# Luh1124/face-vae

Hardware: AMD Instinct MI355X
Metric: training images/sec (256x256 face-VAE step) (higher is better)
Workload: dtype bf16; 1 GPU; FaceVAE step 256x256 (AFE trunk + reparam + Generator trunk, MSE+KL, Adam); global_batch=32, per_gpu_batch=32, resolution=256, parallelism=dp1

## Files before the change

face-vae_amd/csrc/conv.hip:

```cpp
#include "conv_plan.h"

namespace {

#ifdef FV_DIAG
constexpr int DIAG_SLOTS = 8;
__device__ unsigned long long g_diag[4096 * 8 * DIAG_SLOTS];
#define FV_DIAG_T(var) const unsigned long long var = __builtin_amdgcn_s_memtime()
#define FV_DIAG_PUT(slot, val)                                                                     \
  do {                                                                                             \
    const unsigned long long v_ = (val);                                                           \
    if ((threadIdx.x & 63) == 0 && blockIdx.x < 4096)                                              \
      g_diag[((size_t)blockIdx.x * (blockDim.x >> 6) + (threadIdx.x >> 6)) * DIAG_SLOTS + (slot)] = v_; \
  } while (0)
#define FV_DIAG_BEGIN()                                                \
  FV_DIAG_T(d_t0);                                                     \
  const unsigned long long d_r0 = __builtin_amdgcn_s_memrealtime();    \
  unsigned long long d_tw = 0, d_ti = 0, d_wb = 0
#define FV_DIAG_PROLOGUE() FV_DIAG_T(d_t1)
#define FV_DIAG_WAIT_BEGIN() FV_DIAG_T(d_wa)
#define FV_DIAG_WAIT_END()                   \
  do {                                       \
    d_wb = __builtin_amdgcn_s_memtime();     \
    d_tw += d_wb - d_wa;                     \
  } while (0)
// ... 142 lines not shown
  auto bcnt = [&](int j) { return j < nsteps ? (2 * j + 1 < ntap ? 2 : 1) * JB : 0; };
  issue_b(0, 0);
  issue_halo(0);
  if (nch > 1) issue_halo(1);
  for (int i = 1; i < NSB - 1; ++i)
    if (i < nsteps) issue_b(i, i);
  wait_vm<0>();
  __syncthreads();
  FV_DIAG_PROLOGUE();
  int pend = 0;
  if (NSB - 1 < nsteps) {
    issue_b(NSB - 1, NSB - 1);
    pend = bcnt(NSB - 1);
  }
  load_frags(fa0, fb0, 0, 0);
  int hn = 2, hstep = (9 * 2 - 10) / 2;
  int bj = 0;
  for (int j = 0; j + 1 < nsteps; ++j) {
    load_frags(fa1, fb1, 2 * j + 1, bj);
    mfma_all(fa0, fb0);
    const int bn1 = bj + 1 == NSB ? 0 : bj + 1;
    FV_DIAG_WAIT_BEGIN();
    if constexpr (NSB == 2) wait_vm<0>();
    else if (pend == 2 * JB) wait_vm<2 * JB>();
    else wait_vm_dyn(pend);
    wait_lgkm0();
    __builtin_amdgcn_s_barrier();
    asm volatile("" ::: "memory");
    FV_DIAG_WAIT_END();
    if (hn < nch && j == hstep) {
      issue_halo(hn);
      ++hn;
      hstep = (9 * hn - 10) / 2;
    }
    pend = 0;
    if (j + NSB < nsteps) {
      issue_b(j + NSB, bj);
      pend = bcnt(j + NSB);
    }
    load_frags(fa0, fb0, 2 * j + 2, bn1);
    FV_DIAG_ISSUE_END();
    mfma_all(fa1, fb1);
    bj = bn1;
  }
  {
    const int j = nsteps - 1;
    const bool two = 2 * j + 1 < ntap;
    load_frags(fa1, fb1, two ? 2 * j + 1 : 2 * j, bj);
    mfma_all(fa0, fb0);
    if (two) mfma_all(fa1, fb1);
  }
  FV_DIAG_LOOP_END();
  __syncthreads();
  conv_epilogue<bf16, WN, WM, RN, RM, true>(a, acc, smem, co0, p0, tm, wn, wm, lane, tid);
  FV_DIAG_END();
}

template <int WM, int RM, typename Mid = NoMid>
__device__ __forceinline__ void subpix_epilogue(const ConvArgs& a, f32x4 (&acc)[4][RM], char* smem, int tn, int n,
                                                int h0, int w0, int tm, int wn, int wm, int lane, int tid,
                                                Mid mid = Mid{}) {
  constexpr bool kMid = !std::is_same<Mid, NoMid>::value;
  constexpr int RN = 4, NT = 64 * 4 * WM, BN = 256, BM = WM * RM * 16, CPR = BN / 8;
  const int lr = lane & 15, lh = lane >> 4;
  const int cb0 = tn * 64;
#pragma unroll
  for (int nn = 0; nn < RN; ++nn)
#pragma unroll
    for (int i = 0; i < 4; ++i) {
      const int co = cb0 + nn * 16 + lh * 4 + i;
      const float bv = a.bias ? a.bias[co] : 0.f;
#pragma unroll
      for (int m = 0; m < RM; ++m) acc[nn][m][i] += bv;
    }
  if (a.stats) {
    const int rec = (tm * WM + wm) * 4 + wn;
#pragma unroll
    for (int nn = 0; nn < RN; ++nn) {
      float sv[4], qv[4];
#pragma unroll
      for (int i = 0; i < 4; ++i) {
        float t = 0.f, q = 0.f;
#pragma unroll
        for (int m = 0; m < RM; ++m) {
          t += acc[nn][m][i];
          q += acc[nn][m][i] * acc[nn][m][i];
        }
        sv[i] = row16_sum(t);
        qv[i] = row16_sum(q);
      }
      const int cb = cb0 + nn * 16 + lh * 4;
      const int ii = lr & 3;
      const float s01 = ii & 1 ? sv[1] : sv[0], s23 = ii & 1 ? sv[3] : sv[2];
      const float q01 = ii & 1 ? qv[1] : qv[0], q23 = ii & 1 ? qv[3] : qv[2];
      const float val = lr < 4 ? (ii & 2 ? s23 : s01) : (ii & 2 ? q23 : q01);
      if (lr < 8 && rec < a.nrec) a.stats[(long)(rec * 2 + (lr >> 2)) * a.Cout + cb + ii] = val;
    }
  }
  __syncthreads();
#pragma unroll
  for (int nn = 0; nn < RN; ++nn) {
    const int cl = wn * 64 + nn * 16 + lh * 4;
#pragma unroll
    for (int m = 0; m < RM; ++m) {
      const int pl = wm * RM * 16 + m * 16 + lr;
      bf16 t4[4] = {(bf16)acc[nn][m][0], (bf16)acc[nn][m][1], (bf16)acc[nn][m][2], (bf16)acc[nn][m][3]};
      char* dst = smem + pl * BN * 2 + (((cl >> 3) ^ (pl & (CPR - 1))) << 4) + ((cl & 4) << 1);
// ... 205 lines not shown
    auto step_barrier = [&]() {
      FV_DIAG_WAIT_BEGIN();
      if constexpr (NSB == 2) wait_vm<0>();
      else if (pend == 2 * JB) wait_vm<2 * JB>();
      else wait_vm_dyn(pend);
      wait_lgkm0();
      __builtin_amdgcn_s_barrier();
      asm volatile("" ::: "memory");
      FV_DIAG_WAIT_END();
    };
    for (int j = 0; j + 1 < nsteps; ++j) {
      load_frags(fa1, fb1, 2 * j + 1, bj);
      if constexpr ((SCH & 2) != 0) {
        if (stag) step_barrier();
      }
      mfma_all(fa0, fb0);
      const int bn1 = bj + 1 == NSB ? 0 : bj + 1;
      if (!stag) step_barrier();
      if (hn < nch && j == hstep) {
        issue_halo(hn);
        ++hn;
        hstep = halo_step(hn);
      }
      pend = 0;
      if (j + NSB < nsteps) {
        issue_b(t.wbase, j + NSB, bj);
        pend = bcnt(j + NSB);
      }
      load_frags(fa0, fb0, 2 * j + 2, bn1);
      FV_DIAG_ISSUE_END();
      mfma_all(fa1, fb1);
      bj = bn1;
    }
    load_frags(fa1, fb1, 2 * nsteps - 1, bj);
    mfma_all(fa0, fb0);
    mfma_all(fa1, fb1);
    if constexpr (SCH & 1) __builtin_amdgcn_s_setprio(0);
    FV_DIAG_LOOP_END();
    __syncthreads();
    const int vn = v + (int)gridDim.x;
    const bool nxt = PERS && vn < ntl;
    const Tile cur = t;
    if constexpr (PERS) {
      auto mid = [&]() {
        if (nxt) {
          t = tile_of(vn);
          mk_hoff(t);
          issue_prologue(t);
        }
      };
      if constexpr (MODE == 1)
        subpix_epilogue<WM, RM>(a, acc, smem, cur.tn, cur.n, cur.th * TR, cur.tw * 64, cur.tm, wn, wm, lane, tid, mid);
      else
        conv_epilogue<bf16, WN, WM, RN, RM, true>(a, acc, smem, cur.co0, cur.p0, cur.tm, wn, wm, lane, tid, mid);
    } else {
      if constexpr (MODE == 1)
        subpix_epilogue<WM, RM>(a, acc, smem, cur.tn, cur.n, cur.th * TR, cur.tw * 64, cur.tm, wn, wm, lane, tid);
      else
        conv_epilogue<bf16, WN, WM, RN, RM, true>(a, acc, smem, cur.co0, cur.p0, cur.tm, wn, wm, lane, tid);
    }
    FV_DIAG_END();
    if (!nxt) break;
    v = vn;
    first = false;
  }
}

template <int KS, int CIN, int RN, int TR, bool WLDS, bool KSPLIT>
__global__ void __launch_bounds__(512, 4)
conv_halo_fwd(ConvArgs a, unsigned x_bytes) {
  constexpr int PAD = KS / 2, TW = 64;
  constexpr int MT = TR * 4;
  constexpr int RM = KSPLIT ? MT : MT / 8;
  constexpr int HR = TR + KS - 1, HW = TW + KS - 1;
  constexpr int CPP = CIN / 8;
  constexpr int HCH = HR * HW * CPP;
  constexpr int HQ = (HCH + 63) / 64;
  constexpr int KPAD = ((KS * KS * CIN + 31) / 32) * 32;
  constexpr int NKS = KPAD / 32;
  constexpr int KPW = (NKS + 7) / 8;
  constexpr int WROW = KPAD / 8 + 1;
  constexpr int WCH = RN * 16 * WROW;
  constexpr int WQ = WLDS ? (WCH + 63) / 64 : 0;
  constexpr int HB = HQ * 1024, WB = WQ * 1024;
  constexpr int SCR = 4096;
  static_assert(!KSPLIT || (RN == 1 && !WLDS && 8 * MT * 1024 <= HB), "k-split layout");
  __shared__ __attribute__((aligned(1024))) char smem[HB + WB + SCR];
  char* halo = smem;
  char* wlds = smem + HB;

  const int tid = threadIdx.x, lane = tid & 63;
  const int wave = __builtin_amdgcn_readfirstlane(tid >> 6);
  const int tiles_w = a.W / TW, tiles_h = a.H / TR;
  const int tile = blockIdx.x;
  const int n = tile / (tiles_h * tiles_w);
  const int rem = tile - n * tiles_h * tiles_w;
  const int h0 = (rem / tiles_w) * TR, w0 = (rem % tiles_w) * TW;
  const int li = lane & 15, g = lane >> 4;
  const bf16* __restrict__ wk = reinterpret_cast<const bf16*>(a.w);

  const __amdgpu_buffer_rsrc_t xr = __builtin_amdgcn_make_buffer_rsrc(const_cast<void*>(a.x), 0, (int)x_bytes, 0x00020000);
  for (int q = wave; q < HQ; q += 8) {
    const int L = q * 64 + lane;
    const int hp = L / CPP, ch = L - (L / CPP) * CPP;
    const int hr = hp / HW, hc = hp - (hp / HW) * HW;
    const int hh = h0 + hr - PAD, ww = w0 + hc - PAD;
    const int sc = ch ^ (hp & (CPP - 1));
    const bool ok = L < HCH && hh >= 0 && hh < a.H && ww >= 0 && ww < a.W;
    const unsigned off = ok ? (unsigned)((((n * a.H + hh) * a.W + ww) * CIN + sc * 8) * 2) : 0x80000000u;
    dma16(xr, halo + q * 1024, off);
  }
  if constexpr (WLDS) {
// ... 1511 lines not shown
  for (int i = 0; i < n; ++i) {
    const fv_conv_desc* d = &descs[i];
    int st = check_desc(d);
    if (st) return st;
    FV_REQUIRE(d->dtype == dtype, "weight_prep_multi: one dtype per call");
    FV_REQUIRE(fv_conv_weight_prep_batchable(d), "weight_prep_multi: conv %d needs a special layout", i);
    FV_REQUIRE(w_params[i] && wks[i], "weight_prep_multi: null pointer (conv %d)", i);
    const int ks = d->ksize;
    WPrepMJob j0{w_params[i], sigmas[i], wks[i], wrows(d->cout), kpad_lay(smaj_wk(d), kpad_of(ks, d->cin)),
                 fv_ilog2(d->cin),
                 ks * ks * d->cin, 0, 0, d->cout, d->cin_valid, ks, 0, smaj_wk(d)};
    j0.nb = (int)std::min<long>(fv_cdiv((long)j0.rows * j0.Kpad, 256), 256);
    nb_total = std::max(nb_total, j0.nb);
    m.j[m.n++] = j0;
    if (wts[i]) {
      const int cin_t = pad_pow2_8(d->cout);
      WPrepMJob j1{w_params[i], sigmas[i], wts[i], wrows(d->cin), kpad_lay(smaj_wt(d), kpad_of(ks, cin_t)),
                   fv_ilog2(cin_t),
                   ks * ks * cin_t, 1, 0, d->cout, d->cin_valid, ks, 0, smaj_wt(d)};
      j1.nb = (int)std::min<long>(fv_cdiv((long)j1.rows * j1.Kpad, 256), 256);
      nb_total = std::max(nb_total, j1.nb);
      m.j[m.n++] = j1;
    }
  }
  hipStream_t s = (hipStream_t)stream;
  if (dtype == FV_BF16)
    hipLaunchKernelGGL(weight_prep_multi_kernel<bf16>, dim3(nb_total, m.n), dim3(256), 0, s, m);
  else
    hipLaunchKernelGGL(weight_prep_multi_kernel<float>, dim3(nb_total, m.n), dim3(256), 0, s, m);
  return fv_check_launch("weight_prep_multi");
}

static int sr_geometry(const fv_conv_desc* d, int* bp) {
  if (d->dtype != FV_BF16 || use_c7n(d) || halo_tr(d) || use_subpix(d) || use_c64(d)) return 0;
  const int bn = halo3_bn(d);
  const long P = (long)d->n * d->h * d->w;
  if (!bn || d->cout % bn || P % 256) return 0;
  const int nw = bn == 64 ? 4 : 8;
  if (bp) *bp = 256 / nw;
  return (int)(P / 256 * nw);
}

extern "C++" {
static int cu_count() {
  static int n = 0;
  if (!n) {
    int dev = 0;
    if (hipGetDevice(&dev) != hipSuccess || hipDeviceGetAttribute(&n, hipDeviceAttributeMultiprocessorCount, dev) != hipSuccess ||
        n <= 0)
      n = 256;
  }
  return n;
}
template <int WN, int WM, int RN, int RM, int NSB, int MODE>
static void launch_h3(int ntiles, hipStream_t s, const ConvArgs& a, unsigned xb) {
  const int sch = res_sched(2) >= 2 ? 2 : 0;
  const char* e = getenv("FV_PERS_GRID");
  const int cap = (e && atoi(e) > 0) ? atoi(e) : cu_count();
  const bool pers = WN * RN * 16 < 256 && ntiles > cap;
  const dim3 g(pers ? cap : ntiles), b(64 * WN * WM);
  if constexpr (WN * RN * 16 < 256) {
    if (pers) {
      if (sch == 2) hipLaunchKernelGGL((conv3_halo_fwd3<WN, WM, RN, RM, NSB, 2, MODE, true>), g, b, 0, s, a, xb, ntiles);
      else hipLaunchKernelGGL((conv3_halo_fwd3<WN, WM, RN, RM, NSB, 0, MODE, true>), g, b, 0, s, a, xb, ntiles);
      return;
    }
  }
  {
    if (sch == 2) hipLaunchKernelGGL((conv3_halo_fwd3<WN, WM, RN, RM, NSB, 2, MODE, false>), g, b, 0, s, a, xb, ntiles);
    else hipLaunchKernelGGL((conv3_halo_fwd3<WN, WM, RN, RM, NSB, 0, MODE, false>), g, b, 0, s, a, xb, ntiles);
  }
}
}

static bool use_c1s(const fv_conv_desc* d) {
  const char* e = getenv("FV_C1S");
  if (e && e[0] == '0') return false;
  if (!use_v2(d) || d->ksize != 1 || d->upsample || d->pro_act) return false;
  if ((d->cin != 256 && d->cin != 512) || d->cout % 256 || d->ldy != d->cout) return false;
  const long P = (long)d->n * d->h * d->w;
  return P % (32768 / d->cin) == 0 && P * d->cout * 2 < (1L << 31);
}

static int conv_run(const fv_conv_desc* d, const void* x, const void* wk, const float* bias,
                    const float* psc, const float* psh, const void* res, void* y, float* stats,
                    hipStream_t s, const fv_store_reduce* sr = nullptr) {
  ConvArgs a{};
  if (sr && sr->mode) {
    FV_REQUIRE(sr_geometry(d, nullptr) > 0, "store-pass records not available for this conv (query fv_conv2d_sr_records)");
    FV_REQUIRE(sr->records, "store-pass records: null buffer");
    FV_REQUIRE(sr->mode == 1 || (sr->mode == 2 && sr->bn_input && sr->mean && sr->invstd && sr->gamma && sr->beta && !res),
               "store-pass records: bad mode / BN arguments");
    FV_REQUIRE(!stats, "store-pass records and accumulator statistics in one call are not supported");
    a.spm = sr->mode;
    a.sprec = sr->records;
    a.bnm = sr->mean; a.bni = sr->invstd; a.bng = sr->gamma; a.bnb = sr->beta; a.bns = sr->slope;
    if (sr->mode == 2) res = sr->bn_input;
  }
  const FwdTile t = fwd_tile(d->cout);
  a.x = x; a.w = wk; a.bias = bias; a.psc = psc; a.psh = psh; a.slope = d->pro_slope;
  a.res = res; a.y = y; a.stats = stats;
  a.nrec = stats ? fv_conv2d_stats_blocks(d) : 0;
  a.N = d->n; a.H = d->h; a.W = d->w;
  a.Hin = d->upsample ? d->h / 2 : d->h;
  a.Win = d->upsample ? d->w / 2 : d->w;
  a.P = d->n * d->h * d->w;
// ... 56 lines not shown
    const int hl = d->h / 2, wl = d->w / 2;
    const long base = (long)d->n * (wl / 32) * (d->cout / 64);
    int nb = 1;
    while (base * nb < 256 && hl % (nb * 16) == 0) nb *= 2;
    const int nblk = (int)(base * nb);
    const unsigned xb = (unsigned)((long)d->n * hl * wl * 128 * 2);
    hipLaunchKernelGGL(conv3up_band_fwd, dim3(nblk), dim3(512), 0, s, a, xb, nb);
    return fv_check_launch("conv2d_fwd_upband");
  }
  if (use_subpix_halo(d)) {
    FV_REQUIRE(!res && !a.spm, "sub-pixel conv: no residual / store-pass records");
    a.H = a.Hin; a.W = a.Win;
    a.Ho = d->h; a.Wo = d->w;
    a.P = d->n * a.H * a.W;
    a.lgtw = 6;
    a.wus = 4 * d->cout * 64;
    a.ntn = d->cout / 64;
    const int nblk = a.ntn * d->n * (a.H / 4) * (a.W / 64);
    const unsigned xb = (unsigned)((long)d->n * a.H * a.W * d->cin * 2);
    FV_REQUIRE((long)4 * (d->cin / 32) * a.wus / 2 <= phase_wk_elems(d), "sub-pixel halo conv: weight image");
    launch_h3<4, 2, 4, 8, 2, 1>(nblk, s, a, xb);
    return fv_check_launch("conv2d_fwd_subpix_halo");
  }
  if (use_subpix(d)) {
    FV_REQUIRE(!res, "sub-pixel conv: no residual");
    const FwdTile t2 = fwd_tile_v2(d->cout);
    a.H = a.Hin; a.W = a.Win;
    a.Ho = d->h; a.Wo = d->w;
    a.P = d->n * a.H * a.W;
    a.lgw = fv_ilog2(a.W); a.lghw = fv_ilog2(a.H * a.W);
    a.Kpad = kpad_of(2, d->cin);
    a.nks = a.Kpad / BK2;
    a.ntn = fv_cdiv(d->cout, t2.bn);
    a.wphase = wrows(d->cout) * a.Kpad;
    if ((st = wext(4L * a.ntn * t2.bn, a.Kpad, "subpix"))) return st;
    const int nblk2 = 4 * a.ntn * (a.P / t2.bm);
    const long xb = (long)d->n * a.Hin * a.Win * d->cin * 2;
    st = launch_v2(a, 2, t2, 2, nblk2, (unsigned)xb, s);
    if (st) {
      fv_set_error("sub-pixel conv variant unsupported (cout=%d)", d->cout);
      return st;
    }
    return fv_check_launch("conv2d_fwd_subpix");
  }
  if (const int bn = c64 ? 0 : halo3_bn(d)) {
    FV_REQUIRE(!(res && stats), "conv v2: residual and BN statistics in one call are not supported");
    a.lgtw = 6;
    a.wus = wk_rows(d) * 64;
    a.ntn = d->cout / bn;
    if ((st = wext(a.ntn * bn, 9L * d->cin, "halo3")) || (st = wext(wk_rows(d), 9L * d->cin, "halo3 units")))
      return st;
    const int nblk = a.ntn * d->n * (d->h / 4) * (d->w / 64);
    const unsigned xb = (unsigned)((long)d->n * d->h * d->w * d->cin * 2);
    if (bn >= 128 && a.Cin % 64 == 0) {
      if (bn == 256) launch_h3<4, 2, 4, 8, 2, 0>(nblk, s, a, xb);
      else launch_h3<2, 4, 4, 4, 3, 0>(nblk, s, a, xb);
    } else if (bn == 256) {
      hipLaunchKernelGGL((conv3_halo_fwd2<4, 2, 4, 8, 2>), dim3(nblk), dim3(512), 0, s, a, xb);
    } else if (bn == 128) {
      hipLaunchKernelGGL((conv3_halo_fwd2<2, 4, 4, 4, 3>), dim3(nblk), dim3(512), 0, s, a, xb);
    } else if (d->h % 8 == 0 && a.Cin % 64 == 0) {
      const int nblk8 = a.ntn * d->n * (d->h / 8) * (d->w / 64);
      launch_h3<1, 8, 4, 4, 2, 0>(nblk8, s, a, xb);
    } else {
      hipLaunchKernelGGL((conv3_halo_fwd2<1, 4, 4, 4, 3>), dim3(nblk), dim3(256), 0, s, a, xb);
    }
    return fv_check_launch("conv2d_fwd_halo3");
  }
  if (use_c1s(d) && !res && !stats && !a.spm) {
    if ((st = wext(d->cout, a.Kpad, "c1s"))) return st;
    FV_REQUIRE(a.Kpad == d->cin, "1x1 stream conv: K %d != Kpad %d", d->cin, a.Kpad);
    const int ncg = d->cout / 256;
    const int grid = std::max(8 * ncg, cu_count() / (8 * ncg) * (8 * ncg));
    const unsigned xb = (unsigned)((long)a.P * d->cin * 2);
    const char* e = getenv("FV_C1S_BP");
    const bool big = e && atoi(e) == 128;
    if (d->cin == 256) {
      if (big) hipLaunchKernelGGL((conv1x1_stream<256, 128>), dim3(grid), dim3(512), 0, s, a, xb);
      else hipLaunchKernelGGL((conv1x1_stream<256, 64>), dim3(grid), dim3(512), 0, s, a, xb);
    } else {
      if (big) hipLaunchKernelGGL((conv1x1_stream<512, 64>), dim3(grid), dim3(512), 0, s, a, xb);
      else hipLaunchKernelGGL((conv1x1_stream<512, 32>), dim3(grid), dim3(512), 0, s, a, xb);
    }
    return fv_check_launch("conv2d_fwd_c1s");
  }
  if (use_v2(d)) {
    FV_REQUIRE(!(res && stats), "conv v2: residual and BN statistics in one call are not supported");
    const FwdTile t2 = fwd_tile_v2(d->cout);
    a.ntn = fv_cdiv(d->cout, t2.bn);
    a.nks = a.Kpad / BK2;
    if ((st = wext((long)a.ntn * t2.bn, a.Kpad, "v2"))) return st;
    const int nblk2 = a.ntn * fv_cdiv(a.P, t2.bm);
    const long xb = (long)d->n * a.Hin * a.Win * d->cin * 2;
    st = launch_v2(a, d->ksize, t2, d->upsample, nblk2, (unsigned)xb, s);
    if (st) {
      fv_set_error("conv v2 variant unsupported (k=%d ups=%d)", d->ksize, d->upsample);
      return st;
    }
    return fv_check_launch("conv2d_fwd_v2");
  }
  const int nblk = a.ntn * fv_cdiv(a.P, t.bm);
  if ((st = wext((long)a.ntn * t.bn, a.Kpad, "v1"))) return st;
  st = d->dtype == FV_BF16 ? launch_fwd<bf16>(a, d->ksize, t, d->pro_act, d->upsample, nblk, s)
                           : launch_fwd<float>(a, d->ksize, t, d->pro_act, d->upsample, nblk, s);
  if (st) {
    fv_set_error("conv variant unsupported (k=%d pro=%d ups=%d)", d->ksize, d->pro_act, d->upsample);
// ... 42 lines not shown
}

int fv_conv2d_sr_records(const fv_conv_desc* d, int dgrad, int* record_pixels) {
  if (check_desc(d) != FV_OK) return 0;
  if (dgrad) {
    if (d->upsample) return 0;
    const fv_conv_desc t = dgrad_desc(d);
    return sr_geometry(&t, record_pixels);
  }
  return sr_geometry(d, record_pixels);
}

int fv_conv2d_fwd_sr(const fv_conv_desc* d, const void* x, const void* wk, const float* bias, const void* res, void* y,
                     const fv_store_reduce* sr, void* stream) {
  int st = check_desc(d);
  if (st) return st;
  FV_REQUIRE(x && wk && y && sr && sr->mode == 1, "fwd_sr: null pointer or mode != 1");
  FV_REQUIRE(!d->pro_act && !d->out_nchw_f32 && d->ldy == d->cout, "fwd_sr: plain NHWC output only");
  return conv_run(d, x, wk, bias, nullptr, nullptr, res, y, nullptr, (hipStream_t)stream, sr);
}

int fv_conv2d_bwd_data_sr(const fv_conv_desc* d, const void* dy, int ldy_dy, const void* wt, void* dx,
                          const fv_store_reduce* sr, void* stream) {
  int st = check_desc(d);
  if (st) return st;
  FV_REQUIRE(dy && wt && dx && sr && sr->mode == 2 && !d->upsample, "bwd_data_sr: bad argument");
  const fv_conv_desc t = dgrad_desc(d);
  FV_REQUIRE(ldy_dy == t.cin, "bwd_data: dy channel stride must be %d (got %d)", t.cin, ldy_dy);
  return conv_run(&t, dy, wt, nullptr, nullptr, nullptr, nullptr, dx, nullptr, (hipStream_t)stream, sr);
}

int fv_conv2d_bwd_data(const fv_conv_desc* d, const void* dy, int ldy_dy, const void* wt, void* dx,
                       void* stream) {
  int st = check_desc(d);
  if (st) return st;
  const fv_conv_desc t = dgrad_desc(d);
  FV_REQUIRE(ldy_dy == t.cin, "bwd_data: dy channel stride must be %d (got %d)", t.cin, ldy_dy);
  if (const int bn = dgrad_halo_bn(d)) {
    FV_REQUIRE(dy && wt && dx, "null pointer");
    ConvArgs a{};
    a.x = dy; a.w = wt; a.y = dx;
    a.N = d->n; a.H = d->h / 2; a.W = d->w / 2; a.Hin = d->h; a.Win = d->w;
    a.Ho = a.H; a.Wo = a.W;
    a.P = d->n * a.H * a.W;
    a.Cin = 4 * d->cout;
    a.K = d->cout;
    a.Cout = d->cin; a.ldy = d->cin;
    a.lgtw = 6;
    a.wus = d->cin * 64;
    a.ntn = d->cin / bn;
    const int nblk = a.ntn * d->n * (a.H / 4) * (a.W / 64);
    const unsigned xb = (unsigned)((long)d->n * d->h * d->w * d->cout * 2);
    FV_REQUIRE((long)(a.Cin / 32) * 4 * a.wus / 2 <= phase_wt_elems(d), "low-res halo dgrad: weight image");
    if (bn == 256) launch_h3<4, 2, 4, 8, 2, 2>(nblk, (hipStream_t)stream, a, xb);
    else launch_h3<2, 4, 4, 4, 3, 2>(nblk, (hipStream_t)stream, a, xb);
    return fv_check_launch("conv2d_bwd_data_lowres_halo");
  }
  if (use_dgrad_lowres(d)) {
    FV_REQUIRE(dy && wt && dx, "null pointer");
    ConvArgs a{};
    const FwdTile t2 = fwd_tile_v2(d->cin);
    a.x = dy; a.w = wt; a.y = dx;
    a.N = d->n; a.H = d->h / 2; a.W = d->w / 2; a.Hin = d->h; a.Win = d->w;
    a.Ho = a.H; a.Wo = a.W;
    a.P = d->n * a.H * a.W;
    a.Cin = t.cin; a.lgCin = fv_ilog2(t.cin);
    a.Cout = d->cin; a.ldy = d->cin;
    a.Kpad = 16 * t.cin; a.K = a.Kpad; a.nks = a.Kpad / BK2;
    a.ntn = fv_cdiv(d->cin, t2.bn);
    const int nblk = a.ntn * fv_cdiv(a.P, t2.bm);
    const long xb = (long)d->n * d->h * d->w * t.cin * 2;
    const int st = launch_v2(a, 4, t2, 3, nblk, (unsigned)xb, (hipStream_t)stream);
    if (st) {
      fv_set_error("low-res dgrad variant unsupported (cin=%d)", d->cin);
      return st;
    }
    return fv_check_launch("conv2d_bwd_data_lowres");
  }
  return conv_run(&t, dy, wt, nullptr, nullptr, nullptr, nullptr, dx, nullptr, (hipStream_t)stream);
}

int fv_conv2d_wgrad_nsplit(const fv_conv_desc* d) {
  if (check_desc(d) != FV_OK) return 0;
  return plan_wgrad(d).nsplit;
}

size_t fv_conv2d_wgrad_slab_elems(const fv_conv_desc* d) {
  if (check_desc(d) != FV_OK) return 0;
  const WgPlan p = plan_wgrad(d);
  return (size_t)(p.sub ? 4 : 1) * p.nsplit * p.CW * p.KW;
}

size_t fv_conv2d_wgrad_bias_slab_elems(const fv_conv_desc* d) {
  if (check_desc(d) != FV_OK) return 0;
  const WgPlan p = plan_wgrad(d);
  return (size_t)(p.sub ? 4 : 1) * p.nsplit * p.CW;
}

int fv_conv2d_bwd_weight(const fv_conv_desc* d, const void* x, const float* pro_scale,
                         const float* pro_shift, const void* dy, int ldy_dy, float* slab,
                         float* bias_slab, void* stream) {
  int st = check_desc(d);
  if (st) return st;
  FV_REQUIRE(x && dy && slab, "null pointer");
  FV_REQUIRE(ldy_dy % 8 == 0 && ldy_dy >= d->cout, "wgrad: dy channel stride must be a multiple of 8 >= cout");
  FV_REQUIRE(!d->pro_act || (pro_scale && pro_shift), "prologue needs scale/shift");
// ... 1384 lines not shown
```

face-vae_amd/csrc/conv_common.h:

```cpp
#pragma once
#include <stdlib.h>

#include <algorithm>
#include <type_traits>

#include "common.h"

#pragma GCC visibility push(hidden)

struct ConvArgs {
  const void* x;
  const void* w;
  const float* bias;
  const float* psc;
  const float* psh;
  float slope;
  const void* res;
  void* y;
  float* stats;
  int N, H, W, Hin, Win, P;
  int lgCin, Cin;
  int Cout, ldy;
  int K, Kpad, nks;
  int sigmoid, nchw;
// ... 49 lines not shown
}

template <typename T>
__device__ __forceinline__ void load4(const T* p, float* f);
template <>
__device__ __forceinline__ void load4<float>(const float* p, float* f) {
  float4 v = *reinterpret_cast<const float4*>(p);
  f[0] = v.x; f[1] = v.y; f[2] = v.z; f[3] = v.w;
}
template <>
__device__ __forceinline__ void load4<bf16>(const bf16* p, float* f) {
  uint2 v = *reinterpret_cast<const uint2*>(p);
  f[0] = __uint_as_float(v.x << 16); f[1] = __uint_as_float(v.x & 0xffff0000u);
  f[2] = __uint_as_float(v.y << 16); f[3] = __uint_as_float(v.y & 0xffff0000u);
}
template <typename T>
__device__ __forceinline__ void store4(T* p, const float* f);
template <>
__device__ __forceinline__ void store4<float>(float* p, const float* f) {
  *reinterpret_cast<float4*>(p) = make_float4(f[0], f[1], f[2], f[3]);
}
template <>
__device__ __forceinline__ void store4<bf16>(bf16* p, const float* f) {
  bf16 t[4] = {(bf16)f[0], (bf16)f[1], (bf16)f[2], (bf16)f[3]};
  *reinterpret_cast<uint2*>(p) = *reinterpret_cast<const uint2*>(t);
}

template <typename T>
struct Frag;
template <>
struct Frag<bf16> {
  bf16x8 v;
  __device__ __forceinline__ void lds(const char* p) { v = *reinterpret_cast<const bf16x8*>(p); }
};
template <>
struct Frag<float> {
  float v[8];
  __device__ __forceinline__ void lds(const char* p) {
    float4 a = reinterpret_cast<const float4*>(p)[0];
    float4 b = reinterpret_cast<const float4*>(p)[1];
    v[0] = a.x; v[1] = a.y; v[2] = a.z; v[3] = a.w;
    v[4] = b.x; v[5] = b.y; v[6] = b.z; v[7] = b.w;
  }
};
__device__ __forceinline__ f32x4 mma(const Frag<bf16>& a, const Frag<bf16>& b, f32x4 c) {
  return __builtin_amdgcn_mfma_f32_16x16x32_bf16(a.v, b.v, c, 0, 0, 0);
}
__device__ __forceinline__ f32x4 mma(const Frag<float>& a, const Frag<float>& b, f32x4 c) {
#pragma unroll
  for (int j = 0; j < 8; ++j) c = __builtin_amdgcn_mfma_f32_16x16x4f32(a.v[j], b.v[j], c, 0, 0, 0);
  return c;
}

struct NoMid {
  __device__ void operator()() const {}
};
template <typename T, int WN, int WM, int RN, int RM, bool STAGED = false, typename Mid = NoMid, bool GSUB = false>
__device__ __forceinline__ void conv_epilogue(const ConvArgs& a, f32x4 (&acc)[RN][RM], char* smem, int co0, int p0,
                                              int tm, int wn, int wm, int lane, int tid, Mid mid = Mid{}) {
  constexpr bool kMid = !std::is_same<Mid, NoMid>::value;
  constexpr int NT = 64 * WN * WM;
  constexpr int BN = WN * RN * 16;
  constexpr int BM = WM * RM * 16;
  const int HW = a.H * a.W;
  const int lr = lane & 15, lh = lane >> 4;
  constexpr int SCPR = BN / 8, NRES = STAGED ? (BM * SCPR + NT - 1) / NT : 1;
  uint4 rpre[NRES];
  auto load_res = [&]() {
    if (a.res) {
#pragma unroll
      for (int it = 0; it < NRES; ++it) {
        const int idx = tid + it * NT;
        const int pl = idx / SCPR, ch = idx - (idx / SCPR) * SCPR;
        const int tp = a.lgtw ? p0 + (pl >> a.lgtw) * a.W + (pl & ((1 << a.lgtw) - 1)) : p0 + pl;
        const int co = co0 + ch * 8;
        rpre[it] = make_uint4(0, 0, 0, 0);
        if (idx < BM * SCPR && tp < a.P && co < a.Cout)
          rpre[it] = *reinterpret_cast<const uint4*>(reinterpret_cast<const bf16*>(a.res) +
                                                      (long)out_pix<GSUB>(a, tp) * a.ldy + co);
      }
    }
  };
  if constexpr (STAGED && !kMid) load_res();
  float bv[RN][4];
#pragma unroll
  for (int n = 0; n < RN; ++n)
#pragma unroll
    for (int i = 0; i < 4; ++i) {
      const int co = co0 + wn * RN * 16 + n * 16 + lh * 4 + i;
      bv[n][i] = (a.bias && co < a.Cout) ? a.bias[co] : 0.f;
    }
  bool pv[RM];
  int pix_of[RM];
#pragma unroll
  for (int m = 0; m < RM; ++m) {
    const int loc = wm * RM * 16 + m * 16 + lr;
    const int tp = a.lgtw ? p0 + (loc >> a.lgtw) * a.W + (loc & ((1 << a.lgtw) - 1)) : p0 + loc;
    pv[m] = tp < a.P;
    pix_of[m] = out_pix<GSUB>(a, tp);
  }
#pragma unroll
  for (int n = 0; n < RN; ++n) {
    const int cb = co0 + wn * RN * 16 + n * 16 + lh * 4;
#pragma unroll
    for (int m = 0; m < RM; ++m) {
#pragma unroll
      for (int i = 0; i < 4; ++i) acc[n][m][i] += bv[n][i];
      if (!STAGED && a.res && pv[m]) {
        const T* rp = reinterpret_cast<const T*>(a.res) + (long)pix_of[m] * a.ldy + cb;
        if (cb + 3 < a.Cout) {
          float f[4];
          load4<T>(rp, f);
#pragma unroll
          for (int i = 0; i < 4; ++i) acc[n][m][i] += f[i];
        } else {
#pragma unroll
          for (int i = 0; i < 4; ++i)
            if (cb + i < a.Cout) acc[n][m][i] += Elt<T>::to_f(rp[i]);
        }
      }
    }
  }

  const long pout = a.Ho ? (long)a.N * a.Ho * a.Wo : (long)a.P;
  if (a.stats && (long)(tm * WM + wm) < (pout + RM * 16 - 1) / (RM * 16) && tm * WM + wm < a.nrec) {
    const int rec = tm * WM + wm;
#pragma unroll
    for (int n = 0; n < RN; ++n) {
      float sv[4], qv[4];
#pragma unroll
      for (int i = 0; i < 4; ++i) {
        float t = 0.f, q = 0.f;
#pragma unroll
        for (int m = 0; m < RM; ++m) {
          const float v = pv[m] ? acc[n][m][i] : 0.f;
          t += v;
          q += v * v;
        }
        sv[i] = row16_sum(t);
        qv[i] = row16_sum(q);
      }
      const int cb = co0 + wn * RN * 16 + n * 16 + lh * 4;
      const int ii = lr & 3;
      const float s01 = ii & 1 ? sv[1] : sv[0], s23 = ii & 1 ? sv[3] : sv[2];
      const float q01 = ii & 1 ? qv[1] : qv[0], q23 = ii & 1 ? qv[3] : qv[2];
      const float val = lr < 4 ? (ii & 2 ? s23 : s01) : (ii & 2 ? q23 : q01);
      if (lr < 8 && cb + ii < a.Cout) a.stats[(long)(rec * 2 + (lr >> 2)) * a.Cout + cb + ii] = val;
    }
  }

  if constexpr (STAGED) {
    static_assert(sizeof(T) == 2, "staged epilogue is bf16 NHWC");
    constexpr int CPR = BN / 8;
    __syncthreads();
#pragma unroll
    for (int n = 0; n < RN; ++n) {
      const int cl = wn * RN * 16 + n * 16 + lh * 4;
#pragma unroll
      for (int m = 0; m < RM; ++m) {
        const int pl = wm * RM * 16 + m * 16 + lr;
        bf16 t4[4] = {(bf16)acc[n][m][0], (bf16)acc[n][m][1], (bf16)acc[n][m][2], (bf16)acc[n][m][3]};
        char* dst = smem + pl * BN * 2 + (((cl >> 3) ^ (pl & (CPR - 1))) << 4) + ((cl & 4) << 1);
        *reinterpret_cast<uint2*>(dst) = *reinterpret_cast<const uint2*>(t4);
      }
    }
    __syncthreads();
    uint4 vv[kMid ? NRES : 1];
    if constexpr (kMid) {
#pragma unroll
      for (int it = 0; it < NRES; ++it) {
        const int idx = tid + it * NT;
        const int pl = idx / CPR, ch = idx - (idx / CPR) * CPR;
        if (idx < BM * CPR) vv[it] = *reinterpret_cast<const uint4*>(smem + pl * BN * 2 + ((ch ^ (pl & (CPR - 1))) << 4));
      }
      __syncthreads();
      load_res();
      mid();
    }
    auto chunk = [&](int it, int pl, int ch) -> uint4 {
      if constexpr (kMid) return vv[it];
      else return *reinterpret_cast<const uint4*>(smem + pl * BN * 2 + ((ch ^ (pl & (CPR - 1))) << 4));
    };
    if (!a.spm) {
#pragma unroll
      for (int it = 0; it < NRES; ++it) {
        const int idx = tid + it * NT;
        if (idx >= BM * CPR) break;
        const int pl = idx / CPR, ch = idx - (idx / CPR) * CPR;
        const int tp = a.lgtw ? p0 + (pl >> a.lgtw) * a.W + (pl & ((1 << a.lgtw) - 1)) : p0 + pl;
        const int co = co0 + ch * 8;
        if (tp >= a.P || co >= a.Cout) continue;
        const int pix = out_pix<GSUB>(a, tp);
        Chunk8<bf16> v;
        v.raw = chunk(it, pl, ch);
        T* yp = reinterpret_cast<T*>(a.y) + (long)pix * a.ldy + co;
        if (a.res) {
          Chunk8<bf16> r;
          r.raw = rpre[it];
          float f[8];
#pragma unroll
          for (int j = 0; j < 8; ++j) f[j] = v.get(j) + r.get(j);
          v.set8(f);
        }
        v.store(reinterpret_cast<bf16*>(yp));
      }
      return;
    }
    const int sch = tid % CPR;
    float sacc[8], qacc[8], bm_[8], bi_[8], bg_[8], bb_[8];
#pragma unroll
    for (int j = 0; j < 8; ++j) sacc[j] = qacc[j] = 0.f;
    if (a.spm == 2) {
      const int c = co0 + sch * 8;
#pragma unroll
      for (int j = 0; j < 8; ++j) {
        const bool ok = c + j < a.Cout;
        bm_[j] = ok ? a.bnm[c + j] : 0.f;
        bi_[j] = ok ? a.bni[c + j] : 0.f;
        bg_[j] = ok ? a.bng[c + j] : 0.f;
        bb_[j] = ok ? a.bnb[c + j] : 0.f;
      }
    }
#pragma unroll
    for (int it = 0; it < NRES; ++it) {
      const int idx = tid + it * NT;
      if (idx >= BM * CPR) break;
      const int pl = idx / CPR, ch = idx - (idx / CPR) * CPR;
      const int tp = a.lgtw ? p0 + (pl >> a.lgtw) * a.W + (pl & ((1 << a.lgtw) - 1)) : p0 + pl;
      const int co = co0 + ch * 8;
      if (tp >= a.P || co >= a.Cout) continue;
      const int pix = out_pix<GSUB>(a, tp);
      Chunk8<bf16> v;
      v.raw = chunk(it, pl, ch);
      T* yp = reinterpret_cast<T*>(a.y) + (long)pix * a.ldy + co;
      Chunk8<bf16> r;
// ... 143 lines not shown
```

Baseline: 2667 images/s.

## Specialize halo conv epilogue with precomputed addresses and fused store-pass BN statistics

Adds a HALO template path to the staged conv epilogue for whole-tile halo 3x3 convolutions. It precomputes per-thread global and LDS addresses, drops bounds checks, fetches bias once per lane and broadcasts it with ds_bpermute, and folds residual add, BN-backward reductions and per-channel stats into a single store pass using packed float2 math. The goal is less integer address arithmetic and fewer branches in the epilogue. Host-side requirements now reject shapes that are not whole tiles, which could turn previously supported shapes into errors.

Measured after the change: 2715 images/s (median of 6 runs). 1.02x the previous value.

```diff
diff --git a/face-vae_amd/csrc/conv.hip b/face-vae_amd/csrc/conv.hip
--- a/face-vae_amd/csrc/conv.hip
+++ b/face-vae_amd/csrc/conv.hip
@@ -218,7 +218,7 @@
   }
   FV_DIAG_LOOP_END();
   __syncthreads();
-  conv_epilogue<bf16, WN, WM, RN, RM, true>(a, acc, smem, co0, p0, tm, wn, wm, lane, tid);
+  conv_epilogue<bf16, WN, WM, RN, RM, true, NoMid, false, true>(a, acc, smem, co0, p0, tm, wn, wm, lane, tid);
   FV_DIAG_END();
 }
 
@@ -530,12 +530,13 @@
       if constexpr (MODE == 1)
         subpix_epilogue<WM, RM>(a, acc, smem, cur.tn, cur.n, cur.th * TR, cur.tw * 64, cur.tm, wn, wm, lane, tid, mid);
       else
-        conv_epilogue<bf16, WN, WM, RN, RM, true>(a, acc, smem, cur.co0, cur.p0, cur.tm, wn, wm, lane, tid, mid);
+        conv_epilogue<bf16, WN, WM, RN, RM, true, decltype(mid), false, true>(a, acc, smem, cur.co0, cur.p0, cur.tm, wn, wm,
+                                                                              lane, tid, mid);
     } else {
       if constexpr (MODE == 1)
         subpix_epilogue<WM, RM>(a, acc, smem, cur.tn, cur.n, cur.th * TR, cur.tw * 64, cur.tm, wn, wm, lane, tid);
       else
-        conv_epilogue<bf16, WN, WM, RN, RM, true>(a, acc, smem, cur.co0, cur.p0, cur.tm, wn, wm, lane, tid);
+        conv_epilogue<bf16, WN, WM, RN, RM, true, NoMid, false, true>(a, acc, smem, cur.co0, cur.p0, cur.tm, wn, wm, lane, tid);
     }
     FV_DIAG_END();
     if (!nxt) break;
@@ -2153,6 +2154,10 @@
   }
   return n;
 }
+static bool halo_epi_ok(const ConvArgs& a, int bn, int tr) {
+  return a.lgtw == 6 && !a.sub && !a.nchw && a.W % 64 == 0 && a.H % tr == 0 && a.P == a.N * a.H * a.W &&
+         a.ntn * bn == a.Cout && a.ldy >= a.Cout;
+}
 template <int WN, int WM, int RN, int RM, int NSB, int MODE>
 static void launch_h3(int ntiles, hipStream_t s, const ConvArgs& a, unsigned xb) {
   const int sch = res_sched(2) >= 2 ? 2 : 0;
@@ -2315,6 +2320,9 @@
       return st;
     const int nblk = a.ntn * d->n * (d->h / 4) * (d->w / 64);
     const unsigned xb = (unsigned)((long)d->n * d->h * d->w * d->cin * 2);
+    const int tr = (bn == 64 && d->h % 8 == 0 && a.Cin % 64 == 0) ? 8 : 4;
+    FV_REQUIRE(halo_epi_ok(a, bn, tr), "halo 3x3 conv: %dx%d, cout %d is not whole tiles of %d rows x 64 px x %d co", d->h,
+               d->w, d->cout, tr, bn);
     if (bn >= 128 && a.Cin % 64 == 0) {
       if (bn == 256) launch_h3<4, 2, 4, 8, 2, 0>(nblk, s, a, xb);
       else launch_h3<2, 4, 4, 4, 3, 0>(nblk, s, a, xb);
@@ -2463,6 +2471,8 @@
     const int nblk = a.ntn * d->n * (a.H / 4) * (a.W / 64);
     const unsigned xb = (unsigned)((long)d->n * d->h * d->w * d->cout * 2);
     FV_REQUIRE((long)(a.Cin / 32) * 4 * a.wus / 2 <= phase_wt_elems(d), "low-res halo dgrad: weight image");
+    FV_REQUIRE(halo_epi_ok(a, bn, 4), "low-res halo dgrad: %dx%d, cin %d is not whole tiles of 4 rows x 64 px x %d co", a.H,
+               a.W, d->cin, bn);
     if (bn == 256) launch_h3<4, 2, 4, 8, 2, 2>(nblk, (hipStream_t)stream, a, xb);
     else launch_h3<2, 4, 4, 4, 3, 2>(nblk, (hipStream_t)stream, a, xb);
     return fv_check_launch("conv2d_bwd_data_lowres_halo");
diff --git a/face-vae_amd/csrc/conv_common.h b/face-vae_amd/csrc/conv_common.h
--- a/face-vae_amd/csrc/conv_common.h
+++ b/face-vae_amd/csrc/conv_common.h
@@ -125,10 +125,18 @@
   return c;
 }
 
+typedef float f32x2 __attribute__((ext_vector_type(2)));
+__device__ __forceinline__ f32x2 mul_then_add(f32x2 a, f32x2 b, f32x2 c) {
+#pragma clang fp contract(off)
+  const f32x2 p = a * b;
+  return c + p;
+}
+
 struct NoMid {
   __device__ void operator()() const {}
 };
-template <typename T, int WN, int WM, int RN, int RM, bool STAGED = false, typename Mid = NoMid, bool GSUB = false>
+template <typename T, int WN, int WM, int RN, int RM, bool STAGED = false, typename Mid = NoMid, bool GSUB = false,
+          bool HALO = false>
 __device__ __forceinline__ void conv_epilogue(const ConvArgs& a, f32x4 (&acc)[RN][RM], char* smem, int co0, int p0,
                                               int tm, int wn, int wm, int lane, int tid, Mid mid = Mid{}) {
   constexpr bool kMid = !std::is_same<Mid, NoMid>::value;
@@ -138,9 +146,39 @@
   const int HW = a.H * a.W;
   const int lr = lane & 15, lh = lane >> 4;
   constexpr int SCPR = BN / 8, NRES = STAGED ? (BM * SCPR + NT - 1) / NT : 1;
+  constexpr int PS = NT / SCPR;
+  static_assert(!HALO || (STAGED && !GSUB && RN * 16 == 64 && NT % SCPR == 0 && PS <= 64 && 64 % PS == 0 &&
+                          (BM * SCPR) % NT == 0),
+                "halo epilogue: tile geometry");
+  float hbias = 0.f;
+  if constexpr (HALO) {
+    if (a.bias) hbias = a.bias[co0 + wn * 64 + lane];
+  }
+  int htid = tid;
+  if constexpr (HALO) asm volatile("" : "+v"(htid));
+  const int hpl = htid / SCPR, hch = htid % SCPR;
+  const unsigned hvo = HALO ? (unsigned)((hpl * a.ldy + hch * 8) * 2) : 0u;
+  const long hub = HALO ? ((long)p0 * a.ldy + co0) * 2 : 0L;
+  auto haddr = [&](const void* base, int it) -> char* {
+    const int pl = it * PS;
+    const char* ub = reinterpret_cast<const char*>(base) + hub + ((long)(pl >> 6) * a.W + (pl & 63)) * a.ldy * 2;
+    return const_cast<char*>(ub) + hvo;
+  };
+  const int hsw = hch ^ (hpl & (SCPR - 1));
+  int hl[2] = {hpl * BN * 2, hpl * BN * 2 + 65536};
+  if constexpr (HALO && BM * BN * 2 > 65536) asm volatile("" : "+v"(hl[1]));
+  auto hlds = [&](int it) -> int {
+    constexpr int kRow = PS * BN * 2;
+    return (hl[(it * kRow) >> 16] | ((hsw ^ ((it * PS) & (SCPR - 1))) << 4)) + ((it * kRow) & 0xffff);
+  };
   uint4 rpre[NRES];
   auto load_res = [&]() {
-    if (a.res) {
+    if constexpr (HALO) {
+      if (a.res) {
+#pragma unroll
+        for (int it = 0; it < NRES; ++it) rpre[it] = *reinterpret_cast<const uint4*>(haddr(a.res, it));
+      }
+    } else if (a.res) {
 #pragma unroll
       for (int it = 0; it < NRES; ++it) {
         const int idx = tid + it * NT;
@@ -160,8 +198,12 @@
   for (int n = 0; n < RN; ++n)
 #pragma unroll
     for (int i = 0; i < 4; ++i) {
-      const int co = co0 + wn * RN * 16 + n * 16 + lh * 4 + i;
-      bv[n][i] = (a.bias && co < a.Cout) ? a.bias[co] : 0.f;
+      if constexpr (HALO) {
+        bv[n][i] = __int_as_float(__builtin_amdgcn_ds_bpermute((lh * 4 + n * 16 + i) << 2, __float_as_int(hbias)));
+      } else {
+        const int co = co0 + wn * RN * 16 + n * 16 + lh * 4 + i;
+        bv[n][i] = (a.bias && co < a.Cout) ? a.bias[co] : 0.f;
+      }
     }
   bool pv[RM];
   int pix_of[RM];
@@ -169,7 +211,7 @@
   for (int m = 0; m < RM; ++m) {
     const int loc = wm * RM * 16 + m * 16 + lr;
     const int tp = a.lgtw ? p0 + (loc >> a.lgtw) * a.W + (loc & ((1 << a.lgtw) - 1)) : p0 + loc;
-    pv[m] = tp < a.P;
+    pv[m] = HALO || tp < a.P;
     pix_of[m] = out_pix<GSUB>(a, tp);
   }
 #pragma unroll
@@ -218,7 +260,7 @@
       const float s01 = ii & 1 ? sv[1] : sv[0], s23 = ii & 1 ? sv[3] : sv[2];
       const float q01 = ii & 1 ? qv[1] : qv[0], q23 = ii & 1 ? qv[3] : qv[2];
       const float val = lr < 4 ? (ii & 2 ? s23 : s01) : (ii & 2 ? q23 : q01);
-      if (lr < 8 && cb + ii < a.Cout) a.stats[(long)(rec * 2 + (lr >> 2)) * a.Cout + cb + ii] = val;
+      if (lr < 8 && (HALO || cb + ii < a.Cout)) a.stats[(long)(rec * 2 + (lr >> 2)) * a.Cout + cb + ii] = val;
     }
   }
 
@@ -244,7 +286,8 @@
       for (int it = 0; it < NRES; ++it) {
         const int idx = tid + it * NT;
         const int pl = idx / CPR, ch = idx - (idx / CPR) * CPR;
-        if (idx < BM * CPR) vv[it] = *reinterpret_cast<const uint4*>(smem + pl * BN * 2 + ((ch ^ (pl & (CPR - 1))) << 4));
+        if constexpr (HALO) vv[it] = *reinterpret_cast<const uint4*>(smem + hlds(it));
+        else if (idx < BM * CPR) vv[it] = *reinterpret_cast<const uint4*>(smem + pl * BN * 2 + ((ch ^ (pl & (CPR - 1))) << 4));
       }
       __syncthreads();
       load_res();
@@ -252,8 +295,103 @@
     }
     auto chunk = [&](int it, int pl, int ch) -> uint4 {
       if constexpr (kMid) return vv[it];
+      else if constexpr (HALO) return *reinterpret_cast<const uint4*>(smem + hlds(it));
       else return *reinterpret_cast<const uint4*>(smem + pl * BN * 2 + ((ch ^ (pl & (CPR - 1))) << 4));
     };
+    if constexpr (HALO) {
+      static_assert(CPR <= 64 && 64 % CPR == 0, "store-pass records: chunks per row must divide a wave");
+      const int c = co0 + hch * 8;
+      f32x2 sacc[4], qacc[4];
+#pragma unroll
+      for (int k = 0; k < 4; ++k) sacc[k] = qacc[k] = f32x2{0.f, 0.f};
+      auto pass = [&](auto add, auto recs) {
+        constexpr bool ADD = decltype(add)::value;
+        constexpr int REC = decltype(recs)::value;
+        f32x2 bm_[4], bi_[4], bg_[4], bb_[4];
+        if constexpr (REC == 2) {
+#pragma unroll
+          for (int k = 0; k < 4; ++k) {
+            bm_[k] = f32x2{a.bnm[c + 2 * k], a.bnm[c + 2 * k + 1]};
+            bi_[k] = f32x2{a.bni[c + 2 * k], a.bni[c + 2 * k + 1]};
+            bg_[k] = f32x2{a.bng[c + 2 * k], a.bng[c + 2 * k + 1]};
+            bb_[k] = f32x2{a.bnb[c + 2 * k], a.bnb[c + 2 * k + 1]};
+          }
+        }
+#pragma unroll
+        for (int it = 0; it < NRES; ++it) {
+          Chunk8<bf16> v, r;
+          v.raw = chunk(it, 0, 0);
+          if constexpr (ADD || REC == 2) r.raw = rpre[it];
+          if constexpr (REC == 2) {
+#pragma unroll
+            for (int k = 0; k < 4; ++k) {
+              const f32x2 rr = {r.get(2 * k), r.get(2 * k + 1)}, gv = {v.get(2 * k), v.get(2 * k + 1)};
+              const f32x2 yh = (rr - bm_[k]) * bi_[k];
+              const f32x2 t = bg_[k] * yh + bb_[k];
+              const f32x2 gs = gv * a.bns;
+              const f32x2 g = {t.x > 0.f ? gv.x : gs.x, t.y > 0.f ? gv.y : gs.y};
+              sacc[k] += g;
+              if (k < 3) qacc[k] = f32x2{__builtin_fmaf(g.x, yh.x, qacc[k].x), __builtin_fmaf(g.y, yh.y, qacc[k].y)};
+              else qacc[k] = mul_then_add(g, yh, qacc[k]);
+            }
+          } else {
+            if constexpr (ADD) {
+              float f[8];
+#pragma unroll
+              for (int j = 0; j < 8; ++j) f[j] = v.get(j) + r.get(j);
+              v.set8(f);
+            }
+            if constexpr (REC == 1) {
+#pragma unroll
+              for (int k = 0; k < 4; ++k) {
+                const f32x2 o = {v.get(2 * k), v.get(2 * k + 1)};
+                sacc[k] += o;
+                qacc[k] += o * o;
+              }
+            }
+          }
+          v.store(reinterpret_cast<bf16*>(haddr(a.y, it)));
+          if constexpr (REC != 0) {
+#pragma unroll
+            for (int k = 0; k < 4; ++k) asm volatile("" : "+v"(sacc[k]), "+v"(qacc[k]));
+          }
+          __builtin_amdgcn_sched_barrier(0);
+        }
+      };
+      using No = std::false_type;
+      using Yes = std::true_type;
+      if (!a.spm) {
+        if (a.res) pass(Yes{}, std::integral_constant<int, 0>{});
+        else pass(No{}, std::integral_constant<int, 0>{});
+        return;
+      }
+      if (a.spm == 2) pass(No{}, std::integral_constant<int, 2>{});
+      else if (a.res) pass(Yes{}, std::integral_constant<int, 1>{});
+      else pass(No{}, std::integral_constant<int, 1>{});
+      float ssum[8], qsum[8];
+#pragma unroll
+      for (int j = 0; j < 8; ++j) {
+        ssum[j] = sacc[j >> 1][j & 1];
+        qsum[j] = qacc[j >> 1][j & 1];
+      }
+#pragma unroll
+      for (int o = CPR; o < 64; o <<= 1)
+#pragma unroll
+        for (int j = 0; j < 8; ++j) {
+          ssum[j] += __shfl_xor(ssum[j], o, 64);
+          qsum[j] += __shfl_xor(qsum[j], o, 64);
+        }
+      if (lane < CPR) {
+        const long rec = (long)tm * (NT / 64) + (tid >> 6);
+        float* r0 = a.sprec + (rec * 2) * a.Cout + c;
+        float* r1 = a.sprec + (rec * 2 + 1) * a.Cout + c;
+        *reinterpret_cast<float4*>(r0) = make_float4(ssum[0], ssum[1], ssum[2], ssum[3]);
+        *reinterpret_cast<float4*>(r0 + 4) = make_float4(ssum[4], ssum[5], ssum[6], ssum[7]);
+        *reinterpret_cast<float4*>(r1) = make_float4(qsum[0], qsum[1], qsum[2], qsum[3]);
+        *reinterpret_cast<float4*>(r1 + 4) = make_float4(qsum[4], qsum[5], qsum[6], qsum[7]);
+      }
+      return;
+    }
     if (!a.spm) {
 #pragma unroll
       for (int it = 0; it < NRES; ++it) {
```
